# NeuralRevenant/RASSEngine

Measured on NVIDIA B200. Metric: exact top-10 QPS @10M x 1024 (cosine, ids identical to the fp64 CPU oracle), higher is better.
Workload: dtype bf16 scan (fp32 accumulate) + fp64 rerank

## Files before the change

### rassengine_b200/csrc/common.cuh

```cuda
#pragma once
#include <cuda_runtime.h>
#include <cuda_bf16.h>
#include <stdint.h>
#include <stdio.h>
#include <string>
#include <vector>

#include "../../include/rass_b200.h"

#define RASS_WARPS_PER_CTA 8
#define RASS_MAX_K 128
#define RASS_CAND_MAX 2048
#define RASS_GROUP_Q 64
#define RASS_QPAD 256
#define RASS_STREAM_SEG 64
static inline int rass_tc_seg(int k) { return k > 32 ? 512 : 256; }
__host__ __device__ constexpr int rass_tc_keep(int seg) { return seg == 512 ? 128 : seg / 8; }
#define RASS_EXACT_NQ 4
#define RASS_FINISH_THREADS 1024

struct RowMap {
  int64_t base;
  int32_t g, G, blk_log2;
};
// ... 53 lines not shown
  std::vector<int64_t> indptr_host;
  std::vector<float> idf_host;
  std::vector<float> xmin_host, xmax_host;
  bool force_ordered = false;
  bool maxscore = false;
  int* sel_fallback = nullptr;
  std::vector<TextSegment> pending;
  uint32_t* doclen_dev = nullptr;
  uint32_t* gen_dev = nullptr;
  bool has_rewrite = false;
  int doclen_F = 0;
  int64_t doclen_stride = 0;
  std::vector<int64_t> field_vocab;
  std::vector<int64_t> field_last_row;
  bool contiguous_fields = true;
  std::vector<int64_t> field_doc_count, field_sum_ttf;
  std::vector<uint8_t> field_omit_norms;
  int64_t pending_V = 0;
  void* scratch = nullptr;
  size_t scratch_bytes = 0;
};

struct StoreScalars {
  float rho_x;
  float max_xnorm;
  float rho_x8;
};

struct SearchScalars {
  int flagged_n;
  int max_cand;
  int n_certified;
  int finish_done;
  int tile_ctr[2];
};

struct SearchWs {
  SearchScalars* scal = nullptr;
  int q_cap = 0;
  float* q_raw = nullptr;
  float* q_hat = nullptr;
  __nv_bfloat16* q16 = nullptr;
  double* q_norm = nullptr;
  float* q_rho = nullptr;
  int8_t* q8 = nullptr;
  float* q8_scale = nullptr;
  float* q_rho8 = nullptr;
  uint32_t* q_gthr = nullptr;
  size_t pool_entries = 0;
  size_t pool_alloc_entries = 0;
  float* pool_key = nullptr;
  uint32_t* pool_row = nullptr;
  size_t pool_segs = 0;
  size_t pool_alloc_segs = 0;
  float* pool_thr = nullptr;
  int* pool_cnt = nullptr;
  int* flagged = nullptr;
  int* flagged_host = nullptr;
  void* tmap_q = nullptr;
  void* tmap_q2 = nullptr;
  const void* tmap_qbase = nullptr;
  const void* tmap_q2base = nullptr;
  void* tmap_q8 = nullptr;
  const void* tmap_q8base = nullptr;
};

struct VmArray {
  void* base = nullptr;
  size_t reserved = 0, mapped = 0, chunk = 0;
  int device = 0;
  std::vector<unsigned long long> handles;
};
bool vm_available();
bool vm_reserve(VmArray* a, int device, size_t max_bytes, size_t chunk_hint);
int vm_grow(VmArray* a, size_t bytes);
void vm_free(VmArray* a);

struct rass_engine {
  int dim = 0, dim_pad = 0, metric = 0, device = 0;
  uint32_t flags = 0;
  int num_sms = 0;
  int path = RASS_PATH_AUTO;
  int64_t cap = 0, n_rows = 0, n_live = 0;
  RowMap rmap = {0, 0, 1, RASS_SHARD_BLOCK_LOG2};
  struct ShardSet* shards = nullptr;
  float* x32 = nullptr;
  __nv_bfloat16* x16 = nullptr;
  double* norm64 = nullptr;
  float* sa = nullptr;
// ... 201 lines not shown

  __device__ __forceinline__ bool admits_ascending(K k) const { return k > thr_key; }

  __device__ __noinline__ void insert(K k, uint32_t r) {
    if (!entry_better<K>(k, r, thr_key, thr_row)) return;
    const int lane = threadIdx.x & 31;
    int slot = -1;
#pragma unroll
    for (int i = M - 1; i >= 0; --i)
      if (key[i] == thr_key && row[i] == thr_row) slot = i;
    unsigned holders = __ballot_sync(0xffffffffu, slot >= 0);
    int owner = __ffs(holders) - 1;
    if (lane == owner) {
#pragma unroll
      for (int i = 0; i < M; ++i)
        if (i == slot) { key[i] = k; row[i] = r; }
    }
    K wk = key[0];
    uint32_t wr = row[0];
#pragma unroll
    for (int i = 1; i < M; ++i)
      if (entry_better<K>(wk, wr, key[i], row[i])) { wk = key[i]; wr = row[i]; }
#pragma unroll
    for (int m = 16; m >= 1; m >>= 1) {
      K ok = shfl_xor_t(wk, m);
      uint32_t orow = __shfl_xor_sync(0xffffffffu, wr, m);
      if (entry_better<K>(wk, wr, ok, orow)) { wk = ok; wr = orow; }
    }
    thr_key = wk;
    thr_row = wr;
  }
};

template <bool BF16_ROWS>
__device__ __forceinline__ double exact_key_warp(const float* __restrict__ x32, const __nv_bfloat16* __restrict__ x16,
                                                 const double* __restrict__ norm64, uint32_t row, const float* qs,
                                                 double qnorm, int dim_pad, int metric) {
  const int lane = threadIdx.x & 31;
  double acc = 0.0;
  if (BF16_ROWS) {
    const uint4* p = reinterpret_cast<const uint4*>(x16 + (size_t)row * dim_pad);
    for (int j = lane; j < dim_pad / 8; j += 32) {
      uint4 v = __ldg(p + j);
      const uint32_t w[4] = {v.x, v.y, v.z, v.w};
      const float* qq = qs + j * 8;
#pragma unroll
      for (int e = 0; e < 4; ++e) {
        double a = (double)bf16lo(w[e]), b = (double)bf16hi(w[e]);
        double q0 = (double)qq[2 * e], q1 = (double)qq[2 * e + 1];
        if (metric == RASS_METRIC_COSINE) {
          acc = fma(a, q0, acc);
          acc = fma(b, q1, acc);
        } else {
          double d0 = a - q0, d1 = b - q1;
          acc = fma(d0, d0, acc);
          acc = fma(d1, d1, acc);
        }
      }
    }
  } else {
    const float4* p = reinterpret_cast<const float4*>(x32 + (size_t)row * dim_pad);
    for (int j = lane; j < dim_pad / 4; j += 32) {
      float4 v = __ldg(p + j);
      const float4 q = *reinterpret_cast<const float4*>(qs + j * 4);
      if (metric == RASS_METRIC_COSINE) {
        acc = fma((double)v.x, (double)q.x, acc);
        acc = fma((double)v.y, (double)q.y, acc);
        acc = fma((double)v.z, (double)q.z, acc);
        acc = fma((double)v.w, (double)q.w, acc);
      } else {
        double d0 = (double)v.x - (double)q.x, d1 = (double)v.y - (double)q.y;
        double d2 = (double)v.z - (double)q.z, d3 = (double)v.w - (double)q.w;
        acc = fma(d0, d0, acc);
        acc = fma(d1, d1, acc);
        acc = fma(d2, d2, acc);
        acc = fma(d3, d3, acc);
      }
    }
  }
  acc = warp_sum(acc);
  if (metric == RASS_METRIC_COSINE) {
    double den = norm64[row] * qnorm;
    return den > 0.0 ? acc / den : 0.0;
  }
  return -acc;
}

__device__ __forceinline__ float int8_key(int32_t acc1, int32_t acc2, float s1, float s2, float sa8, float sb) {
  return __fmaf_rn(__fmaf_rn(s1, __int2float_rn(acc1), __fmul_rn(s2, __int2float_rn(acc2))), sa8, sb);
}

__device__ __forceinline__ float warp_max_nonneg(float v) {
  return __uint_as_float(__reduce_max_sync(0xffffffffu, __float_as_uint(v)));
}

__device__ __forceinline__ float int8_code(float v, float s) {
  return s > 0.f ? fminf(fmaxf(rintf(__fdiv_rn(v, s)), -127.f), 127.f) : 0.f;
}

__device__ __forceinline__ float score_from_key(double key, int metric) {
  return metric == RASS_METRIC_COSINE ? (float)(1.0 / (2.0 - key)) : (float)(1.0 / (1.0 - key));
}

#endif

int launch_store_convert(rass_engine* h, const float* src_dev, int64_t src_stride, int64_t first_row, int64_t n,
                         cudaStream_t st);
int launch_query_prep(rass_engine* h, const SearchWs& ws, const float* q_dev, int B, cudaStream_t st);
int launch_seed_thresholds(rass_engine* h, const SearchWs& ws, int B, int seg, size_t n_clear, bool* cleared,
// ... 104 lines not shown
```

### rassengine_b200/csrc/engine.cu

```cuda
#include <stdarg.h>
#include <string.h>

#include <algorithm>

#include "common.cuh"

thread_local std::string g_create_error;

int rass_fail(rass_engine* h, int code, const char* fmt, ...) {
  char buf[512];
  va_list ap;
  va_start(ap, fmt);
  vsnprintf(buf, sizeof(buf), fmt, ap);
  va_end(ap);
  if (h) h->err = buf;
  else g_create_error = buf;
  return code;
}

extern "C" const char* rass_version(void) { return "rass-b200 0.1 (abi 1, sm_100a)"; }

extern "C" const char* rass_last_error(const rass_engine* h) { return h ? h->err.c_str() : g_create_error.c_str(); }

#define CHECK_HANDLE(h)                    \
// ... 119 lines not shown
  do {                                                                                              \
    cudaError_t e_ = (call);                                                                        \
    if (e_ != cudaSuccess) {                                                                        \
      h->err = std::string(#call) + " failed: " + cudaGetErrorString(e_);                           \
      return bail(e_ == cudaErrorMemoryAllocation ? RASS_E_OOM : RASS_E_CUDA);                      \
    }                                                                                               \
  } while (0)
  CREATE_TRY(cudaStreamCreateWithFlags(&h->stream, cudaStreamNonBlocking));
  CREATE_TRY(cudaStreamCreateWithFlags(&h->copy_stream, cudaStreamNonBlocking));
  for (int i = 0; i < 4; ++i) CREATE_TRY(cudaEventCreate(&h->ev[i]));
  for (int i = 0; i < 2; ++i) CREATE_TRY(cudaEventCreateWithFlags(&h->stage_ev[i], cudaEventDisableTiming));
  h->stage_bytes = (size_t)32 << 20;
  for (int i = 0; i < 2; ++i) CREATE_TRY(cudaMallocHost(&h->stage[i], h->stage_bytes));
  CREATE_TRY(cudaMalloc(&h->store_scal, sizeof(StoreScalars)));
  CREATE_TRY(cudaMemset(h->store_scal, 0, sizeof(StoreScalars)));
  CREATE_TRY(cudaMalloc(&h->ws[0].scal, sizeof(SearchScalars)));
  CREATE_TRY(cudaMemset(h->ws[0].scal, 0, sizeof(SearchScalars)));
  CREATE_TRY(cudaMallocHost(&h->scal_host, sizeof(SearchScalars)));
  memset(h->scal_host, 0, sizeof(SearchScalars));
#undef CREATE_TRY
  if (capacity_rows > 0) {
    int rc = ensure_capacity(h, capacity_rows);
    if (rc) return bail(rc);
  }
  *out = h;
  return RASS_OK;
}

static void free_search_ws(SearchWs& w) {
  cudaFree(w.scal);
  cudaFree(w.q_raw); cudaFree(w.q_hat); cudaFree(w.q16); cudaFree(w.q_norm); cudaFree(w.q_rho); cudaFree(w.q_gthr);
  cudaFree(w.q8); cudaFree(w.q8_scale); cudaFree(w.q_rho8);
  cudaFree(w.pool_key); cudaFree(w.pool_row); cudaFree(w.pool_thr); cudaFree(w.pool_cnt);
  cudaFree(w.flagged); cudaFreeHost(w.flagged_host);
  free(w.tmap_q); free(w.tmap_q2); free(w.tmap_q8);
}

extern "C" int rass_destroy(rass_engine* h) {
  SHARDED(h, sharded_destroy(h));
  if (!h) return RASS_OK;
  cudaSetDevice(h->device);
  cudaDeviceSynchronize();
  if (h->use_vm) {
    for (int i = 0; i < 7; ++i) vm_free(&h->vm[i]);
  } else {
    cudaFree(h->x32); cudaFree(h->x16); cudaFree(h->norm64); cudaFree(h->sa); cudaFree(h->sb);
    cudaFree(h->x8); cudaFree(h->sa8);
  }
  cudaFree(h->store_scal); cudaFreeHost(h->scal_host);
  for (SearchWs& w : h->ws) free_search_ws(w);
  cudaFree(h->dev_stage);
  cudaFree(h->xlist_key); cudaFree(h->xlist_row);
  cudaFree(h->out_rows); cudaFree(h->out_scores); cudaFree(h->out_keys);
  cudaFreeHost(h->out_rows_host); cudaFreeHost(h->out_scores_host); cudaFreeHost(h->out_keys_host);
  cudaFreeHost(h->q_stage_host);
  cudaFree(h->q_stage_dev);
  cudaFree(h->row_filter);
  cudaFree(h->filter_rows_dev);
  cudaFree(h->flist_dev);
  cudaFree(h->sb_filtered);
  cudaFree(h->retry_ids); cudaFree(h->retry_q); cudaFree(h->retry_rows); cudaFree(h->retry_scores); cudaFree(h->retry_keys);
  for (int i = 0; i < 2; ++i) {
    if (h->slot_stream[i]) cudaStreamDestroy(h->slot_stream[i]);
    if (h->slot_fork[i]) cudaEventDestroy(h->slot_fork[i]);
  }
  for (cudaEvent_t e : h->ev_pool) if (e) cudaEventDestroy(e);
// ... 374 lines not shown
  REALLOC_DEV(h, ws.q_norm, cap);
  REALLOC_DEV(h, ws.q_rho, cap);
  REALLOC_DEV(h, ws.q_gthr, cap);
  if (has_int8_shadow(h->flags)) {
    REALLOC_DEV(h, ws.q8, cap * 2 * d);
    REALLOC_DEV(h, ws.q8_scale, cap * 2);
    REALLOC_DEV(h, ws.q_rho8, cap);
  }
  REALLOC_DEV(h, ws.flagged, cap);
  REALLOC_HOST(h, ws.flagged_host, cap);
  ws.q_cap = (int)cap;
  ws.tmap_qbase = nullptr;
  ws.tmap_q2base = nullptr;
  ws.tmap_q8base = nullptr;
  return RASS_OK;
}

int ensure_pool(rass_engine* h, SearchWs& ws, size_t entries_per_query, size_t segs_per_query, size_t n_queries) {
  const size_t need_e = entries_per_query * n_queries, need_s = segs_per_query * n_queries;
  if (need_e > ws.pool_alloc_entries) {
    { const int rc_ = sync_for_realloc(h); if (rc_) return rc_; }
    ws.pool_alloc_entries = 0;
    REALLOC_DEV(h, ws.pool_key, need_e);
    REALLOC_DEV(h, ws.pool_row, need_e);
    ws.pool_alloc_entries = need_e;
  }
  if (need_s > ws.pool_alloc_segs) {
    { const int rc_ = sync_for_realloc(h); if (rc_) return rc_; }
    ws.pool_alloc_segs = 0;
    REALLOC_DEV(h, ws.pool_thr, need_s);
    REALLOC_DEV(h, ws.pool_cnt, need_s);
    ws.pool_alloc_segs = need_s;
  }
  ws.pool_entries = entries_per_query;
  ws.pool_segs = segs_per_query;
  return RASS_OK;
}

int ensure_xlist_workspace(rass_engine* h, size_t entries) {
  if (entries <= h->xlist_entries) return RASS_OK;
  CUDA_TRY(h, cudaStreamSynchronize(eng_stream(h)));
  REALLOC_DEV(h, h->xlist_key, entries * RASS_EXACT_NQ);
  REALLOC_DEV(h, h->xlist_row, entries * RASS_EXACT_NQ);
  h->xlist_entries = entries;
  return RASS_OK;
}

int ensure_out_workspace(rass_engine* h, size_t n) {
  if (n <= h->out_cap) return RASS_OK;
  CUDA_TRY(h, cudaStreamSynchronize(eng_stream(h)));
  REALLOC_DEV(h, h->out_rows, n);
  REALLOC_DEV(h, h->out_scores, n);
  REALLOC_DEV(h, h->out_keys, n);
  REALLOC_HOST(h, h->out_rows_host, n);
  REALLOC_HOST(h, h->out_scores_host, n);
  REALLOC_HOST(h, h->out_keys_host, n);
  h->out_cap = n;
  return RASS_OK;
}

__global__ void fill_empty_kernel(int64_t* rows, float* scores, double* keys, size_t n) {
  const size_t i = (size_t)blockIdx.x * blockDim.x + threadIdx.x;
  if (i >= n) return;
  rows[i] = -1;
  scores[i] = 0.f;
  if (keys) keys[i] = 0.0;
// ... 126 lines not shown
    s.n_certified = B;
    s.launches = 1;
    if (stats) *stats = s;
    return RASS_OK;
  }
  if ((rc = refresh_store_scalars(h))) return rc;
  int path = resolve_path(h, B, k);
  int64_t* flag_out = as ? async_flag_dev : nullptr;
  if (robust && (path == RASS_PATH_STREAM || path == RASS_PATH_UMMA8)) path = RASS_PATH_UMMA;
  s.path = path;
  if (!(as && h->async_overlap) && (rc = select_scan_offsets(h, st))) return rc;
  if (!as) CUDA_TRY(h, cudaEventRecord(h->ev[0], st));
  if ((rc = launch_query_prep(h, ws, q_dev, B, st))) return rc;
  s.launches = 1;
  size_t n_ev = 0;
  if (path == RASS_PATH_EXACT) {
    for (int i = 0; i < B; ++i) ws.flagged_host[i] = i;
    CUDA_TRY(h, cudaEventRecord(h->ev[1], st));
    if ((rc = launch_exact(h, ws, k, ws.flagged_host, B, out_rows, out_scores, out_keys, st, &s.launches))) return rc;
    s.n_fallback = B;
    s.passes = (B + RASS_EXACT_NQ - 1) / RASS_EXACT_NQ;
    s.bytes_streamed = (int64_t)s.passes * h->n_rows * h->dim_pad * ((h->flags & RASS_BF16_ONLY) ? 2 : 4);
  } else if (path == RASS_PATH_GEMM) {
    const int n_segs = scan_gemm_segs(h, B);
    const int seg = robust ? rass_tc_seg(k) : 256;
    if ((rc = ensure_pool(h, ws, (size_t)n_segs * seg, (size_t)n_segs, (size_t)B))) return rc;
    bool cleared = false;
    if ((rc = launch_seed_thresholds(h, ws, B, seg, (size_t)n_segs * B, &cleared, st))) return rc;
    CUDA_TRY(h, cudaEventRecord(get_event(h, ev_base + n_ev++), st));
    if ((rc = launch_scan_gemm(h, ws, B, seg, st, cleared))) return rc;
    CUDA_TRY(h, cudaEventRecord(get_event(h, ev_base + n_ev++), st));
    if ((rc = launch_finish(h, ws, 0, B, k, n_segs, seg, true, SCAN_BF16, out_rows, out_scores, out_keys, st, flag_out)))
      return rc;
    s.launches += cleared ? 3 : 4;
    s.passes = (B + 255) / 256;
    s.bytes_streamed = (int64_t)s.passes * h->n_rows * h->dim_pad * 2;
  } else {
    const bool int8 = path == RASS_PATH_UMMA8;
    const bool umma = path == RASS_PATH_UMMA || int8;
    const ScanOperands ops = int8 ? SCAN_INT8 : (umma ? SCAN_BF16 : SCAN_FP32_Q);
    const int n_segs = umma ? scan_umma_segs(h) : scan_stream_segs(h);
    const int seg = umma ? (robust ? rass_tc_seg(k) : 256) : RASS_STREAM_SEG;
    if ((rc = ensure_pool(h, ws, (size_t)n_segs * seg, (size_t)n_segs))) return rc;
    bool cleared = false;
    if (umma) {
      if ((rc = launch_seed_thresholds(h, ws, B, seg, (size_t)n_segs * RASS_GROUP_Q, &cleared, st, int8))) return rc;
      s.launches += 1;
    }
    for (int g0 = 0; g0 < B; g0 += RASS_GROUP_Q) {
      const int ng = std::min(RASS_GROUP_Q, B - g0);
      CUDA_TRY(h, cudaEventRecord(get_event(h, ev_base + n_ev++), st));
      if (umma) {
        const bool skip_clear = cleared && g0 == 0;
        if ((rc = launch_scan_umma(h, ws, g0, ng, seg, st, skip_clear, int8))) return rc;
        s.launches += skip_clear ? 1 : 2;
        s.passes += 1;
      } else {
        for (int q0 = g0; q0 < g0 + ng; q0 += 2) {
          if ((rc = launch_scan_stream(h, ws, q0, std::min(2, g0 + ng - q0), g0, st))) return rc;
          s.launches += 1;
          s.passes += 1;
        }
      }
      CUDA_TRY(h, cudaEventRecord(get_event(h, ev_base + n_ev++), st));
      if ((rc = launch_finish(h, ws, g0, ng, k, n_segs, seg, true, ops, out_rows, out_scores, out_keys, st, flag_out)))
        return rc;
      s.launches += 1;
    }
    s.bytes_streamed = (int64_t)s.passes * h->n_rows * h->dim_pad * (int8 ? 1 : 2);
  }
  if (as) {
    if (path == RASS_PATH_EXACT) return rass_fail(h, RASS_E_INVALID, "the fp64 scan has no async form");
    CUDA_TRY(h, cudaMemcpyAsync(as->scal_host, ws.scal, sizeof(SearchScalars), cudaMemcpyDeviceToHost, st));
    CUDA_TRY(h, cudaEventRecord(as->done, st));
    as->stats = s;
    as->k = k;
    as->n_ev = n_ev;
    as->trivial = false;
    as->pending = true;
    return RASS_OK;
  }
  if (path != RASS_PATH_EXACT) {
    CUDA_TRY(h, cudaEventRecord(h->ev[1], st));
    CUDA_TRY(h, cudaMemcpyAsync(h->scal_host, ws.scal, sizeof(SearchScalars), cudaMemcpyDeviceToHost, st));
    CUDA_TRY(h, cudaStreamSynchronize(st));
    const int nf = h->scal_host->flagged_n;
    note_int8_outcome(h, s.path, B, k, nf, robust);
    s.n_certified = h->scal_host->n_certified;
    s.max_candidates = h->scal_host->max_cand;
    if (nf > 0) {
      CUDA_TRY(h, cudaMemcpyAsync(ws.flagged_host, ws.flagged, (size_t)nf * sizeof(int), cudaMemcpyDeviceToHost, st));
      CUDA_TRY(h, cudaStreamSynchronize(st));
      std::sort(ws.flagged_host, ws.flagged_host + nf);
      const bool second_chance = !robust && (path == RASS_PATH_UMMA8 || (k > 32 && rass_tc_seg(k) != 256));
      if (second_chance) {
        float pre = 0.f;
        CUDA_TRY(h, cudaEventElapsedTime(&pre, h->ev[0], h->ev[1]));
        if ((rc = scan_ms_of(h, ev_base, n_ev, &first_scan_ms))) return rc;
        n_ev = 0;
        first_total_ms = pre;
// ... 363 lines not shown
```

### rassengine_b200/csrc/finish.cu

```cuda
#include "common.cuh"

struct FinishArgs {
  const float* pool_key;
  const uint32_t* pool_row;
  const float* pool_thr;
  const int* pool_cnt;
  size_t pool_entries;
  int n_segs, seg_size;
  const float* x32;
  const __nv_bfloat16* x16;
  const double* norm64;
  const float* q_raw;
  const double* q_norm;
  const float* q_rho;
  const StoreScalars* store;
  int int8;
  SearchScalars* scal;
  int* flagged;
  int dim_pad, metric, k, g0;
  float acc_eps;
  RowMap rmap;
  int64_t* out_rows;
  float* out_scores;
  double* out_keys;
  int64_t* flag_out;
};

template <bool BF16_ROWS>
__global__ void __launch_bounds__(RASS_FINISH_THREADS, 1) finish_kernel(FinishArgs a) {
  extern __shared__ __align__(16) unsigned char smem_raw[];
  float* qs = reinterpret_cast<float*>(smem_raw);
  double* ckey = reinterpret_cast<double*>(qs + a.dim_pad);
  uint32_t* crow = reinterpret_cast<uint32_t*>(ckey + RASS_CAND_MAX);
  __shared__ float s_red[32];
  __shared__ int s_redi[32];
  __shared__ float s_t;
  __shared__ int s_valid, s_ncand, s_have;
  __shared__ double s_sk;

  const int tid = threadIdx.x, lane = tid & 31, warp = tid >> 5;
  const int slot = blockIdx.x;
  const int q = a.g0 + slot;
  const float* pk = a.pool_key + (size_t)slot * a.pool_entries;
  const uint32_t* pr = a.pool_row + (size_t)slot * a.pool_entries;

  for (int j = tid; j < a.dim_pad; j += blockDim.x) qs[j] = a.q_raw[(size_t)q * a.dim_pad + j];
  if (tid == 0) { s_ncand = 0; s_have = 0; }

  float mx = neg_inf<float>();
  int nvalid = 0;
  for (int sgm = warp; sgm < a.n_segs; sgm += RASS_FINISH_THREADS / 32) {
    const int cnt = a.pool_cnt ? min(a.pool_cnt[(size_t)slot * a.n_segs + sgm], a.seg_size) : a.seg_size;
    for (int i = lane; i < cnt; i += 32) {
      const size_t o = (size_t)sgm * a.seg_size + i;
      if (a.pool_cnt || pr[o] != 0xffffffffu) {
        ++nvalid;
        mx = fmaxf(mx, pk[o]);
      }
    }
  }
  float t = neg_inf<float>();
  for (int s = tid; s < a.n_segs; s += blockDim.x) t = fmaxf(t, a.pool_thr[(size_t)slot * a.n_segs + s]);
#pragma unroll
  for (int m = 16; m >= 1; m >>= 1) {
    t = fmaxf(t, __shfl_xor_sync(0xffffffffu, t, m));
    nvalid += __shfl_xor_sync(0xffffffffu, nvalid, m);
  }
  if (lane == 0) { s_red[warp] = t; s_redi[warp] = nvalid; }
  __syncthreads();
  if (warp == 0) {
    float tt = s_red[lane];
    int nv = s_redi[lane];
#pragma unroll
    for (int m = 16; m >= 1; m >>= 1) {
      tt = fmaxf(tt, __shfl_xor_sync(0xffffffffu, tt, m));
      nv += __shfl_xor_sync(0xffffffffu, nv, m);
    }
    if (lane == 0) { s_t = tt; s_valid = nv; }
  }

  float bprime;
  {
    const uint32_t mine = mx > neg_inf<float>() ? ord32(mx) : 0u;
    uint32_t prefix = 0;
#pragma unroll 1
    for (int bit = 31; bit >= 0; --bit) {
      const uint32_t cand = prefix | (1u << bit);
      if (__syncthreads_count(mine >= cand) >= a.k) prefix = cand;
    }
    bprime = prefix > 0x007fffffu ? unord32(prefix) : neg_inf<float>();
  }

  float eps;
  {
    const float rho_x = a.int8 ? a.store->rho_x8 : (BF16_ROWS ? 0.f : a.store->rho_x);
    const float rho_q = a.q_rho ? a.q_rho[q] : 0.f;
    float e = rho_x * (1.f + rho_q) + rho_q + a.acc_eps;
    if (a.metric == RASS_METRIC_L2) {
      const float xm = a.store->max_xnorm;
      e = e * xm * (float)a.q_norm[q] * 1.0001f + 6.0e-8f * xm * xm;
    }
    eps = e * 1.0001f;
  }
  const float cutoff = bprime - 2.f * eps;

  for (int sgm = warp; sgm < a.n_segs; sgm += RASS_FINISH_THREADS / 32) {
    const int cnt = a.pool_cnt ? min(a.pool_cnt[(size_t)slot * a.n_segs + sgm], a.seg_size) : a.seg_size;
    for (int i = lane; i < cnt; i += 32) {
      const size_t o = (size_t)sgm * a.seg_size + i;
      if ((a.pool_cnt || pr[o] != 0xffffffffu) && pk[o] >= cutoff) {
        int pos = atomicAdd(&s_ncand, 1);
        if (pos < RASS_CAND_MAX) crow[pos] = pr[o];
      }
    }
  }
  __syncthreads();
  const int ncand_raw = s_ncand;
  const int ncand = min(ncand_raw, RASS_CAND_MAX);

  const double qn = a.q_norm[q];
  for (int c = warp; c < ncand; c += RASS_FINISH_THREADS / 32) {
    double key = exact_key_warp<BF16_ROWS>(a.x32, a.x16, a.norm64, crow[c], qs, qn, a.dim_pad, a.metric);
    if (lane == 0) ckey[c] = key;
  }
  __syncthreads();

  const int kk = a.k;
  for (int c = tid; c < ncand; c += blockDim.x) {
    const double key = ckey[c];
    const uint32_t row = crow[c];
    int rank = 0;
    for (int j = 0; j < ncand; ++j) rank += entry_better<double>(ckey[j], crow[j], key, row);
    if (rank < kk) {
      const size_t o = (size_t)q * kk + rank;
      a.out_rows[o] = row_local_to_global(a.rmap, (int64_t)row);
      a.out_scores[o] = score_from_key(key, a.metric);
      if (a.out_keys) a.out_keys[o] = a.metric == RASS_METRIC_COSINE ? key : -key;
      if (rank == kk - 1) { s_sk = key; s_have = 1; }
    }
  }
  for (int r = ncand + tid; r < kk; r += blockDim.x) {
    const size_t o = (size_t)q * kk + r;
    a.out_rows[o] = -1;
    a.out_scores[o] = 0.f;
    if (a.out_keys) a.out_keys[o] = 0.0;
  }
  __syncthreads();

  if (tid == 0) {
    bool ok;
    const float tt = s_t;
    if (ncand_raw > RASS_CAND_MAX) {
      ok = false;
    } else if (!s_have) {
      ok = (tt == neg_inf<float>()) && ncand == s_valid;
    } else if (tt == neg_inf<float>()) {
      ok = true;
    } else {
      double sk = s_sk;
      if (a.metric == RASS_METRIC_L2) sk = 0.5 * (qn * qn + sk);
      ok = (double)tt + (double)eps < sk;
    }
    if (ok) {
      atomicAdd(&a.scal->n_certified, 1);
    } else {
      int pos = atomicAdd(&a.scal->flagged_n, 1);
      a.flagged[pos] = q;
    }
    atomicMax(&a.scal->max_cand, ncand_raw);
    if (a.flag_out) {
      __threadfence();
      if (atomicAdd(&a.scal->finish_done, 1) == (int)gridDim.x - 1) {
        a.scal->finish_done = 0;
        *a.flag_out = (int64_t)atomicAdd(&a.scal->flagged_n, 0);
      }
    }
  }
}

static size_t finish_smem(int dim_pad) {
  return (size_t)dim_pad * 4 + RASS_CAND_MAX * 12;
}

int launch_finish(rass_engine* h, const SearchWs& ws, int g0, int ng, int k, int n_segs, int seg_size, bool has_cnt,
                  ScanOperands ops, int64_t* out_rows, float* out_scores, double* out_keys, cudaStream_t st,
                  int64_t* flag_out) {
  FinishArgs a;
  a.flag_out = flag_out;
  a.pool_key = ws.pool_key;
  a.pool_row = ws.pool_row;
  a.pool_thr = ws.pool_thr;
  a.pool_cnt = has_cnt ? ws.pool_cnt : nullptr;
  a.pool_entries = ws.pool_entries;
  a.n_segs = n_segs;
  a.seg_size = seg_size;
  a.x32 = h->x32;
  a.x16 = h->x16;
  a.norm64 = h->norm64;
  a.q_raw = ws.q_raw;
  a.q_norm = ws.q_norm;
  a.q_rho = ops == SCAN_INT8 ? ws.q_rho8 : (ops == SCAN_BF16 ? ws.q_rho : nullptr);
  a.int8 = ops == SCAN_INT8;
  a.store = h->store_scal;
  a.scal = ws.scal;
  a.flagged = ws.flagged;
  a.dim_pad = h->dim_pad;
  a.metric = h->metric;
  a.k = k;
  a.g0 = g0;
  a.acc_eps = acc_allowance(h->dim_pad);
  a.rmap = h->rmap;
  a.out_rows = out_rows;
  a.out_scores = out_scores;
  a.out_keys = out_keys;
  const size_t smem = finish_smem(h->dim_pad);
  if (h->flags & RASS_BF16_ONLY) {
    CUDA_TRY(h, cudaFuncSetAttribute(finish_kernel<true>, cudaFuncAttributeMaxDynamicSharedMemorySize, (int)smem));
    finish_kernel<true><<<ng, RASS_FINISH_THREADS, smem, st>>>(a);
  } else {
    CUDA_TRY(h, cudaFuncSetAttribute(finish_kernel<false>, cudaFuncAttributeMaxDynamicSharedMemorySize, (int)smem));
    finish_kernel<false><<<ng, RASS_FINISH_THREADS, smem, st>>>(a);
  }
  CUDA_TRY(h, cudaGetLastError());
  return RASS_OK;
}

template <bool BF16_ROWS, int M>
__global__ void __launch_bounds__(RASS_WARPS_PER_CTA * 32) exact_scan_kernel(
    const float* __restrict__ x32, const __nv_bfloat16* __restrict__ x16, const double* __restrict__ norm64,
    const float* __restrict__ sb, const float* __restrict__ q_raw, const double* __restrict__ q_norm,
    const int* __restrict__ qids, int nq, int64_t n_rows, int dim_pad, int metric, double* __restrict__ xkey,
    uint32_t* __restrict__ xrow, size_t xlist_entries) {
  extern __shared__ __align__(16) unsigned char smem_raw[];
  float* qs = reinterpret_cast<float*>(smem_raw);
  const int lane = threadIdx.x & 31, warp = threadIdx.x >> 5;
  const int gw = blockIdx.x * RASS_WARPS_PER_CTA + warp;
  const int W = gridDim.x * RASS_WARPS_PER_CTA;
  for (int i = threadIdx.x; i < nq * dim_pad; i += blockDim.x)
    qs[i] = q_raw[(size_t)qids[i / dim_pad] * dim_pad + (i % dim_pad)];
  __syncthreads();
  double qn[RASS_EXACT_NQ];
  WarpTop<double, M> top[RASS_EXACT_NQ];
#pragma unroll
  for (int i = 0; i < RASS_EXACT_NQ; ++i) {
    top[i].init();
    qn[i] = i < nq ? q_norm[qids[i]] : 0.0;
  }
  for (int64_t row = gw; row < n_rows; row += W) {
    if (sb[row] == neg_inf<float>()) continue;
#pragma unroll
    for (int i = 0; i < RASS_EXACT_NQ; ++i) {
      if (i < nq) {
        double key = exact_key_warp<BF16_ROWS>(x32, x16, norm64, (uint32_t)row, qs + (size_t)i * dim_pad, qn[i],
                                               dim_pad, metric);
        if (top[i].admits_ascending(key)) top[i].insert(key, (uint32_t)row);
      }
    }
  }
#pragma unroll
  for (int i = 0; i < RASS_EXACT_NQ; ++i) {
    if (i < nq) {
      const size_t base = (size_t)i * xlist_entries + (size_t)gw * (32 * M);
#pragma unroll
      for (int s = 0; s < M; ++s) {
        xkey[base + s * 32 + lane] = top[i].key[s];
        xrow[base + s * 32 + lane] = top[i].row[s];
      }
    }
  }
}

__device__ __forceinline__ uint64_t ord64(double d) {
  if (d == 0.0) d = 0.0;
  uint64_t u = (uint64_t)__double_as_longlong(d);
  return (u >> 63) ? ~u : (u | 0x8000000000000000ULL);
}

__global__ void __launch_bounds__(1024, 1) exact_select_kernel(const double* __restrict__ xkey,
                                                               const uint32_t* __restrict__ xrow, size_t xlist_entries,
                                                               int n, int k, const int* __restrict__ qids, int q_fixed,
                                                               int raw_score, int metric,
                                                               RowMap rmap, int64_t* __restrict__ out_rows,
                                                               float* __restrict__ out_scores,
                                                               double* __restrict__ out_keys,
                                                               const int* __restrict__ only_if) {
  if (only_if && !only_if[blockIdx.x]) return;
  __shared__ int hist[256];
  __shared__ int s_bucket, s_remaining, s_nsel, s_nvalid;
  __shared__ double selk[RASS_MAX_K];
  __shared__ uint32_t selr[RASS_MAX_K];
  const int tid = threadIdx.x;
  const int q = qids ? qids[blockIdx.x] : q_fixed + (int)blockIdx.x;
  const double* key = xkey + (size_t)blockIdx.x * xlist_entries;
  const uint32_t* row = xrow + (size_t)blockIdx.x * xlist_entries;

  if (tid == 0) { s_nvalid = 0; s_nsel = 0; }
  __syncthreads();
  int nv = 0;
  for (int i = tid; i < n; i += blockDim.x) nv += row[i] != 0xffffffffu;
  if (nv) atomicAdd(&s_nvalid, nv);
  __syncthreads();
  const int kk = min(k, s_nvalid);

  uint64_t pre_hi = 0, mask_hi = 0;
  uint32_t pre_lo = 0, mask_lo = 0;
  if (kk > 0) {
    if (tid == 0) s_remaining = kk;
    for (int byte = 11; byte >= 0; --byte) {
// ... 178 lines not shown
```

### rassengine_b200/csrc/store.cu

```cuda
#include <cooperative_groups.h>

#include "common.cuh"

__global__ void __launch_bounds__(256) store_convert_kernel(const float* __restrict__ src, int64_t src_stride, int dim,
                                                            int dim_pad, int metric, int bf16_only, int write32,
                                                            float* __restrict__ x32, __nv_bfloat16* __restrict__ x16,
                                                            double* __restrict__ norm64, float* __restrict__ sa,
                                                            float* __restrict__ sb, int8_t* __restrict__ x8,
                                                            float* __restrict__ sa8, StoreScalars* scal,
                                                            int64_t first_row, int64_t n) {
  const int lane = threadIdx.x & 31;
  const int64_t r = (int64_t)blockIdx.x * (blockDim.x >> 5) + (threadIdx.x >> 5);
  if (r >= n) return;
  const int64_t row = first_row + r;
  const float* s = src + r * src_stride;
  double n2 = 0.0, e2 = 0.0;
  float amax = 0.f;
  for (int j = lane * 4; j < dim_pad; j += 128) {
    float v[4];
#pragma unroll
    for (int e = 0; e < 4; ++e) {
      v[e] = (j + e < dim) ? s[j + e] : 0.f;
      amax = fmaxf(amax, fabsf(v[e]));
    }
// ... 55 lines not shown
    atomicMax(reinterpret_cast<int*>(&scal->rho_x8), __float_as_int(rho));
  }
}

int launch_store_convert(rass_engine* h, const float* src_dev, int64_t src_stride, int64_t first_row, int64_t n,
                         cudaStream_t st) {
  if (n <= 0) return RASS_OK;
  h->sb_filtered_dirty = true;
  h->store_scal_stale = true;
  const bool bf16_only = (h->flags & RASS_BF16_ONLY) != 0;
  const bool in_place = !bf16_only && src_dev == h->x32 + (size_t)first_row * h->dim_pad;
  const int warps = 8;
  int64_t blocks = (n + warps - 1) / warps;
  store_convert_kernel<<<(unsigned)blocks, warps * 32, 0, st>>>(src_dev, src_stride, h->dim, h->dim_pad, h->metric,
                                                                bf16_only ? 1 : 0, (!bf16_only && !in_place) ? 1 : 0,
                                                                h->x32, h->x16, h->norm64, h->sa, h->sb, h->x8, h->sa8,
                                                                h->store_scal, first_row, n);
  CUDA_TRY(h, cudaGetLastError());
  return RASS_OK;
}

__global__ void __launch_bounds__(128) query_prep_kernel(const float* __restrict__ q, int dim, int dim_pad, int metric,
                                                         int B, int B_pad, float* __restrict__ q_raw,
                                                         float* __restrict__ q_hat, __nv_bfloat16* __restrict__ q16,
                                                         double* __restrict__ q_norm, float* __restrict__ q_rho,
                                                         int8_t* __restrict__ q8, float* __restrict__ q8_scale,
                                                         float* __restrict__ q_rho8, SearchScalars* __restrict__ scal) {
  const int lane = threadIdx.x & 31;
  const int b = blockIdx.x * (blockDim.x >> 5) + (threadIdx.x >> 5);
  if (blockIdx.x == 0 && threadIdx.x == 0) {
    scal->flagged_n = 0;
    scal->max_cand = 0;
    scal->n_certified = 0;
    scal->tile_ctr[0] = 0;
    scal->tile_ctr[1] = 0;
  }
  if (b >= B_pad) return;
  const size_t r1 = (size_t)(b / RASS_GROUP_Q) * (2 * RASS_GROUP_Q) + (b % RASS_GROUP_Q), r2 = r1 + RASS_GROUP_Q;
  if (b >= B) {
    for (int j = lane; j < dim_pad; j += 32) q16[(size_t)b * dim_pad + j] = __float2bfloat16_rn(0.f);
    if (q8) {
      for (int j = lane; j < dim_pad; j += 32) { q8[r1 * dim_pad + j] = 0; q8[r2 * dim_pad + j] = 0; }
      if (lane < 2) q8_scale[2 * b + lane] = 0.f;
    }
    return;
  }
  const float* s = q + (size_t)b * dim;
  double n2 = 0.0;
  for (int j = lane; j < dim; j += 32) n2 = fma((double)s[j], (double)s[j], n2);
  n2 = warp_sum(n2);
  const double nrm = sqrt(n2);
  const double inv = (metric == RASS_METRIC_COSINE) ? (nrm > 0.0 ? 1.0 / nrm : 0.0) : 1.0;
  double h2 = 0.0, e2 = 0.0;
  float amax = 0.f;
  for (int j = lane; j < dim_pad; j += 32) {
    float v = j < dim ? s[j] : 0.f;
    float hat = (float)((double)v * inv);
    amax = fmaxf(amax, fabsf(hat));
    __nv_bfloat16 hb = __float2bfloat16_rn(hat);
    double d = (double)hat - (double)__bfloat162float(hb);
    h2 = fma((double)hat, (double)hat, h2);
    e2 = fma(d, d, e2);
    q_raw[(size_t)b * dim_pad + j] = v;
    q_hat[(size_t)b * dim_pad + j] = hat;
    q16[(size_t)b * dim_pad + j] = hb;
  }
// ... 245 lines not shown
```

Measured before the change: 35270.

## Split finish into collect, grid-wide rerank, and radix select kernels

The single per-query finish kernel becomes three kernels. The first collects candidate rows per query into a global list. The second spreads the fp64 exact-key rerank of all candidates across every SM, instead of tying it to one 1024-thread CTA per query. The third does a radix threshold select followed by ranking only the survivors, replacing an O(ncand^2) rank. The exact-key loop also batches 8 loads per lane and the exact scan gets a min-blocks launch bound, at the cost of two extra launches and global candidate buffers.

Measured after the change: 35530, median of 6. Within noise of the previous version (+0.7%).

```diff
diff --git a/rassengine_b200/csrc/common.cuh b/rassengine_b200/csrc/common.cuh
--- a/rassengine_b200/csrc/common.cuh
+++ b/rassengine_b200/csrc/common.cuh
@@ -109,7 +109,16 @@
   int max_cand;
   int n_certified;
   int finish_done;
+  int cand_total;
   int tile_ctr[2];
+};
+
+struct FinishQuery {
+  float t;
+  float eps;
+  int valid;
+  int ncand;
+  int base;
 };
 
 struct SearchWs {
@@ -132,6 +141,10 @@
   size_t pool_alloc_segs = 0;
   float* pool_thr = nullptr;
   int* pool_cnt = nullptr;
+  size_t cand_slots = 0;
+  uint2* cand_list = nullptr;
+  double* cand_key = nullptr;
+  FinishQuery* cand_q = nullptr;
   int* flagged = nullptr;
   int* flagged_host = nullptr;
   void* tmap_q = nullptr;
@@ -399,6 +412,7 @@
   }
 };
 
+#define EXACT_KEY_LOADS 8
 template <bool BF16_ROWS>
 __device__ __forceinline__ double exact_key_warp(const float* __restrict__ x32, const __nv_bfloat16* __restrict__ x16,
                                                  const double* __restrict__ norm64, uint32_t row, const float* qs,
@@ -407,41 +421,59 @@
   double acc = 0.0;
   if (BF16_ROWS) {
     const uint4* p = reinterpret_cast<const uint4*>(x16 + (size_t)row * dim_pad);
-    for (int j = lane; j < dim_pad / 8; j += 32) {
-      uint4 v = __ldg(p + j);
-      const uint32_t w[4] = {v.x, v.y, v.z, v.w};
-      const float* qq = qs + j * 8;
-#pragma unroll
-      for (int e = 0; e < 4; ++e) {
-        double a = (double)bf16lo(w[e]), b = (double)bf16hi(w[e]);
-        double q0 = (double)qq[2 * e], q1 = (double)qq[2 * e + 1];
-        if (metric == RASS_METRIC_COSINE) {
-          acc = fma(a, q0, acc);
-          acc = fma(b, q1, acc);
-        } else {
-          double d0 = a - q0, d1 = b - q1;
-          acc = fma(d0, d0, acc);
-          acc = fma(d1, d1, acc);
+    const int n = dim_pad / 8;
+    for (int j0 = lane; j0 < n; j0 += 32 * EXACT_KEY_LOADS) {
+      uint4 v[EXACT_KEY_LOADS];
+#pragma unroll
+      for (int u = 0; u < EXACT_KEY_LOADS; ++u)
+        if (j0 + 32 * u < n) v[u] = __ldg(p + j0 + 32 * u);
+#pragma unroll
+      for (int u = 0; u < EXACT_KEY_LOADS; ++u) {
+        const int j = j0 + 32 * u;
+        if (j >= n) break;
+        const uint32_t w[4] = {v[u].x, v[u].y, v[u].z, v[u].w};
+        const float* qq = qs + j * 8;
+#pragma unroll
+        for (int e = 0; e < 4; ++e) {
+          double a = (double)bf16lo(w[e]), b = (double)bf16hi(w[e]);
+          double q0 = (double)qq[2 * e], q1 = (double)qq[2 * e + 1];
+          if (metric == RASS_METRIC_COSINE) {
+            acc = fma(a, q0, acc);
+            acc = fma(b, q1, acc);
+          } else {
+            double d0 = a - q0, d1 = b - q1;
+            acc = fma(d0, d0, acc);
+            acc = fma(d1, d1, acc);
+          }
         }
       }
     }
   } else {
     const float4* p = reinterpret_cast<const float4*>(x32 + (size_t)row * dim_pad);
-    for (int j = lane; j < dim_pad / 4; j += 32) {
-      float4 v = __ldg(p + j);
-      const float4 q = *reinterpret_cast<const float4*>(qs + j * 4);
-      if (metric == RASS_METRIC_COSINE) {
-        acc = fma((double)v.x, (double)q.x, acc);
-        acc = fma((double)v.y, (double)q.y, acc);
-        acc = fma((double)v.z, (double)q.z, acc);
-        acc = fma((double)v.w, (double)q.w, acc);
-      } else {
-        double d0 = (double)v.x - (double)q.x, d1 = (double)v.y - (double)q.y;
-        double d2 = (double)v.z - (double)q.z, d3 = (double)v.w - (double)q.w;
-        acc = fma(d0, d0, acc);
-        acc = fma(d1, d1, acc);
-        acc = fma(d2, d2, acc);
-        acc = fma(d3, d3, acc);
+    const int n = dim_pad / 4;
+    for (int j0 = lane; j0 < n; j0 += 32 * EXACT_KEY_LOADS) {
+      float4 v[EXACT_KEY_LOADS];
+#pragma unroll
+      for (int u = 0; u < EXACT_KEY_LOADS; ++u)
+        if (j0 + 32 * u < n) v[u] = __ldg(p + j0 + 32 * u);
+#pragma unroll
+      for (int u = 0; u < EXACT_KEY_LOADS; ++u) {
+        const int j = j0 + 32 * u;
+        if (j >= n) break;
+        const float4 q = *reinterpret_cast<const float4*>(qs + j * 4);
+        if (metric == RASS_METRIC_COSINE) {
+          acc = fma((double)v[u].x, (double)q.x, acc);
+          acc = fma((double)v[u].y, (double)q.y, acc);
+          acc = fma((double)v[u].z, (double)q.z, acc);
+          acc = fma((double)v[u].w, (double)q.w, acc);
+        } else {
+          double d0 = (double)v[u].x - (double)q.x, d1 = (double)v[u].y - (double)q.y;
+          double d2 = (double)v[u].z - (double)q.z, d3 = (double)v[u].w - (double)q.w;
+          acc = fma(d0, d0, acc);
+          acc = fma(d1, d1, acc);
+          acc = fma(d2, d2, acc);
+          acc = fma(d3, d3, acc);
+        }
       }
     }
   }
diff --git a/rassengine_b200/csrc/engine.cu b/rassengine_b200/csrc/engine.cu
--- a/rassengine_b200/csrc/engine.cu
+++ b/rassengine_b200/csrc/engine.cu
@@ -175,6 +175,7 @@
   cudaFree(w.q_raw); cudaFree(w.q_hat); cudaFree(w.q16); cudaFree(w.q_norm); cudaFree(w.q_rho); cudaFree(w.q_gthr);
   cudaFree(w.q8); cudaFree(w.q8_scale); cudaFree(w.q_rho8);
   cudaFree(w.pool_key); cudaFree(w.pool_row); cudaFree(w.pool_thr); cudaFree(w.pool_cnt);
+  cudaFree(w.cand_list); cudaFree(w.cand_key); cudaFree(w.cand_q);
   cudaFree(w.flagged); cudaFreeHost(w.flagged_host);
   free(w.tmap_q); free(w.tmap_q2); free(w.tmap_q8);
 }
@@ -615,6 +616,14 @@
     REALLOC_DEV(h, ws.pool_cnt, need_s);
     ws.pool_alloc_segs = need_s;
   }
+  if (n_queries > ws.cand_slots) {
+    { const int rc_ = sync_for_realloc(h); if (rc_) return rc_; }
+    ws.cand_slots = 0;
+    REALLOC_DEV(h, ws.cand_list, n_queries * RASS_CAND_MAX);
+    REALLOC_DEV(h, ws.cand_key, n_queries * RASS_CAND_MAX);
+    REALLOC_DEV(h, ws.cand_q, n_queries);
+    ws.cand_slots = n_queries;
+  }
   ws.pool_entries = entries_per_query;
   ws.pool_segs = segs_per_query;
   return RASS_OK;
@@ -807,7 +816,7 @@
     CUDA_TRY(h, cudaEventRecord(get_event(h, ev_base + n_ev++), st));
     if ((rc = launch_finish(h, ws, 0, B, k, n_segs, seg, true, SCAN_BF16, out_rows, out_scores, out_keys, st, flag_out)))
       return rc;
-    s.launches += cleared ? 3 : 4;
+    s.launches += cleared ? 5 : 6;
     s.passes = (B + 255) / 256;
     s.bytes_streamed = (int64_t)s.passes * h->n_rows * h->dim_pad * 2;
   } else {
@@ -840,7 +849,7 @@
       CUDA_TRY(h, cudaEventRecord(get_event(h, ev_base + n_ev++), st));
       if ((rc = launch_finish(h, ws, g0, ng, k, n_segs, seg, true, ops, out_rows, out_scores, out_keys, st, flag_out)))
         return rc;
-      s.launches += 1;
+      s.launches += 3;
     }
     s.bytes_streamed = (int64_t)s.passes * h->n_rows * h->dim_pad * (int8 ? 1 : 2);
   }
diff --git a/rassengine_b200/csrc/finish.cu b/rassengine_b200/csrc/finish.cu
--- a/rassengine_b200/csrc/finish.cu
+++ b/rassengine_b200/csrc/finish.cu
@@ -15,42 +15,50 @@
   const float* q_rho;
   const StoreScalars* store;
   int int8;
+  int bf16_rows;
   SearchScalars* scal;
   int* flagged;
   int dim_pad, metric, k, g0;
   float acc_eps;
   RowMap rmap;
+  uint2* cand_list;
+  double* cand_key;
+  FinishQuery* cand_q;
   int64_t* out_rows;
   float* out_scores;
   double* out_keys;
   int64_t* flag_out;
 };
 
-template <bool BF16_ROWS>
-__global__ void __launch_bounds__(RASS_FINISH_THREADS, 1) finish_kernel(FinishArgs a) {
-  extern __shared__ __align__(16) unsigned char smem_raw[];
-  float* qs = reinterpret_cast<float*>(smem_raw);
-  double* ckey = reinterpret_cast<double*>(qs + a.dim_pad);
-  uint32_t* crow = reinterpret_cast<uint32_t*>(ckey + RASS_CAND_MAX);
+__device__ __forceinline__ uint64_t ord64(double d) {
+  if (d == 0.0) d = 0.0;
+  uint64_t u = (uint64_t)__double_as_longlong(d);
+  return (u >> 63) ? ~u : (u | 0x8000000000000000ULL);
+}
+
+__global__ void __launch_bounds__(RASS_FINISH_THREADS, 1) finish_collect_kernel(FinishArgs a) {
+  __shared__ uint32_t crow[RASS_CAND_MAX];
   __shared__ float s_red[32];
   __shared__ int s_redi[32];
   __shared__ float s_t;
-  __shared__ int s_valid, s_ncand, s_have;
-  __shared__ double s_sk;
+  __shared__ int s_valid, s_ncand, s_base;
 
   const int tid = threadIdx.x, lane = tid & 31, warp = tid >> 5;
   const int slot = blockIdx.x;
   const int q = a.g0 + slot;
   const float* pk = a.pool_key + (size_t)slot * a.pool_entries;
   const uint32_t* pr = a.pool_row + (size_t)slot * a.pool_entries;
-
-  for (int j = tid; j < a.dim_pad; j += blockDim.x) qs[j] = a.q_raw[(size_t)q * a.dim_pad + j];
-  if (tid == 0) { s_ncand = 0; s_have = 0; }
+  auto seg_count = [&](int sgm) {
+    return sgm >= a.n_segs ? 0 : (a.pool_cnt ? min(a.pool_cnt[(size_t)slot * a.n_segs + sgm], a.seg_size) : a.seg_size);
+  };
+
+  if (tid == 0) s_ncand = 0;
 
   float mx = neg_inf<float>();
   int nvalid = 0;
+  int cnt = seg_count(warp);
   for (int sgm = warp; sgm < a.n_segs; sgm += RASS_FINISH_THREADS / 32) {
-    const int cnt = a.pool_cnt ? min(a.pool_cnt[(size_t)slot * a.n_segs + sgm], a.seg_size) : a.seg_size;
+    const int cnt_next = seg_count(sgm + RASS_FINISH_THREADS / 32);
     for (int i = lane; i < cnt; i += 32) {
       const size_t o = (size_t)sgm * a.seg_size + i;
       if (a.pool_cnt || pr[o] != 0xffffffffu) {
@@ -58,6 +66,7 @@
         mx = fmaxf(mx, pk[o]);
       }
     }
+    cnt = cnt_next;
   }
   float t = neg_inf<float>();
   for (int s = tid; s < a.n_segs; s += blockDim.x) t = fmaxf(t, a.pool_thr[(size_t)slot * a.n_segs + s]);
@@ -93,7 +102,7 @@
 
   float eps;
   {
-    const float rho_x = a.int8 ? a.store->rho_x8 : (BF16_ROWS ? 0.f : a.store->rho_x);
+    const float rho_x = a.int8 ? a.store->rho_x8 : (a.bf16_rows ? 0.f : a.store->rho_x);
     const float rho_q = a.q_rho ? a.q_rho[q] : 0.f;
     float e = rho_x * (1.f + rho_q) + rho_q + a.acc_eps;
     if (a.metric == RASS_METRIC_L2) {
@@ -104,8 +113,9 @@
   }
   const float cutoff = bprime - 2.f * eps;
 
+  cnt = seg_count(warp);
   for (int sgm = warp; sgm < a.n_segs; sgm += RASS_FINISH_THREADS / 32) {
-    const int cnt = a.pool_cnt ? min(a.pool_cnt[(size_t)slot * a.n_segs + sgm], a.seg_size) : a.seg_size;
+    const int cnt_next = seg_count(sgm + RASS_FINISH_THREADS / 32);
     for (int i = lane; i < cnt; i += 32) {
       const size_t o = (size_t)sgm * a.seg_size + i;
       if ((a.pool_cnt || pr[o] != 0xffffffffu) && pk[o] >= cutoff) {
@@ -113,30 +123,114 @@
         if (pos < RASS_CAND_MAX) crow[pos] = pr[o];
       }
     }
-  }
-  __syncthreads();
-  const int ncand_raw = s_ncand;
+    cnt = cnt_next;
+  }
+  __syncthreads();
+  const int ncand = min(s_ncand, RASS_CAND_MAX);
+  if (tid == 0) {
+    s_base = atomicAdd(&a.scal->cand_total, ncand);
+    a.cand_q[slot] = FinishQuery{s_t, eps, s_valid, s_ncand, s_base};
+    atomicMax(&a.scal->max_cand, s_ncand);
+  }
+  __syncthreads();
+  for (int i = tid; i < ncand; i += blockDim.x) a.cand_list[s_base + i] = make_uint2(crow[i], (uint32_t)slot);
+}
+
+#define RASS_RERANK_THREADS 256
+#define RASS_RERANK_CTAS_PER_SM 4
+template <bool BF16_ROWS>
+__global__ void __launch_bounds__(RASS_RERANK_THREADS, RASS_RERANK_CTAS_PER_SM) finish_rerank_kernel(FinishArgs a) {
+  constexpr int WARPS = RASS_RERANK_THREADS / 32;
+  const int lane = threadIdx.x & 31;
+  const int n = a.scal->cand_total;
+  const int per_cta = (n + (int)gridDim.x - 1) / (int)gridDim.x;
+  const int end = min(n, ((int)blockIdx.x + 1) * per_cta);
+  int i = (int)blockIdx.x * per_cta + (threadIdx.x >> 5);
+  uint2 next = i < end ? a.cand_list[i] : make_uint2(0, 0);
+  for (; i < end; i += WARPS) {
+    const uint2 cur = next;
+    if (i + WARPS < end) next = a.cand_list[i + WARPS];
+    const int q = a.g0 + (int)cur.y;
+    const double key = exact_key_warp<BF16_ROWS>(a.x32, a.x16, a.norm64, cur.x, a.q_raw + (size_t)q * a.dim_pad,
+                                                 a.q_norm[q], a.dim_pad, a.metric);
+    if (lane == 0) a.cand_key[i] = key;
+  }
+}
+
+#define RASS_SELECT_THREADS 256
+__global__ void __launch_bounds__(RASS_SELECT_THREADS) finish_select_kernel(FinishArgs a) {
+  constexpr int E = RASS_CAND_MAX / RASS_SELECT_THREADS;
+  constexpr int WARPS = RASS_SELECT_THREADS / 32;
+  static_assert(E * RASS_SELECT_THREADS == RASS_CAND_MAX, "every candidate has one thread");
+  __shared__ double skey[RASS_CAND_MAX];
+  __shared__ uint32_t srow[RASS_CAND_MAX];
+  __shared__ int s_cnt[2][WARPS];
+  __shared__ int s_nsel, s_have;
+  __shared__ double s_sk;
+
+  const int tid = threadIdx.x, lane = tid & 31, warp = tid >> 5;
+  const int slot = blockIdx.x, q = a.g0 + slot;
+  const FinishQuery fq = a.cand_q[slot];
+  const int ncand_raw = fq.ncand;
   const int ncand = min(ncand_raw, RASS_CAND_MAX);
-
-  const double qn = a.q_norm[q];
-  for (int c = warp; c < ncand; c += RASS_FINISH_THREADS / 32) {
-    double key = exact_key_warp<BF16_ROWS>(a.x32, a.x16, a.norm64, crow[c], qs, qn, a.dim_pad, a.metric);
-    if (lane == 0) ckey[c] = key;
-  }
-  __syncthreads();
-
   const int kk = a.k;
-  for (int c = tid; c < ncand; c += blockDim.x) {
-    const double key = ckey[c];
-    const uint32_t row = crow[c];
+
+  double key[E];
+  uint32_t row[E];
+  uint64_t ok[E];
+#pragma unroll
+  for (int e = 0; e < E; ++e) {
+    const int i = tid + e * RASS_SELECT_THREADS;
+    key[e] = 0.0;
+    row[e] = 0;
+    ok[e] = 0;
+    if (i < ncand) {
+      key[e] = a.cand_key[fq.base + i];
+      row[e] = a.cand_list[fq.base + i].x;
+      ok[e] = ord64(key[e]);
+    }
+  }
+  if (tid == 0) { s_nsel = 0; s_have = 0; }
+  __syncthreads();
+
+  uint64_t T = 0;
+  int have = ncand;
+#pragma unroll 1
+  for (int bit = 63; bit >= 0 && have > kk; --bit) {
+    const uint64_t c = T | (1ull << bit);
+    int m = 0;
+#pragma unroll
+    for (int e = 0; e < E; ++e) m += ok[e] >= c;
+    m = __reduce_add_sync(0xffffffffu, m);
+    if (lane == 0) s_cnt[bit & 1][warp] = m;
+    __syncthreads();
+    int cnt = 0;
+#pragma unroll
+    for (int w = 0; w < WARPS; ++w) cnt += s_cnt[bit & 1][w];
+    if (cnt >= kk) { T = c; have = cnt; }
+  }
+#pragma unroll
+  for (int e = 0; e < E; ++e) {
+    if (ok[e] != 0 && ok[e] >= T) {
+      const int pos = atomicAdd(&s_nsel, 1);
+      skey[pos] = key[e];
+      srow[pos] = row[e];
+    }
+  }
+  __syncthreads();
+
+  const int nsel = s_nsel;
+  for (int c = tid; c < nsel; c += blockDim.x) {
+    const double kc = skey[c];
+    const uint32_t rc = srow[c];
     int rank = 0;
-    for (int j = 0; j < ncand; ++j) rank += entry_better<double>(ckey[j], crow[j], key, row);
+    for (int j = 0; j < nsel; ++j) rank += entry_better<double>(skey[j], srow[j], kc, rc);
     if (rank < kk) {
       const size_t o = (size_t)q * kk + rank;
-      a.out_rows[o] = row_local_to_global(a.rmap, (int64_t)row);
-      a.out_scores[o] = score_from_key(key, a.metric);
-      if (a.out_keys) a.out_keys[o] = a.metric == RASS_METRIC_COSINE ? key : -key;
-      if (rank == kk - 1) { s_sk = key; s_have = 1; }
+      a.out_rows[o] = row_local_to_global(a.rmap, (int64_t)rc);
+      a.out_scores[o] = score_from_key(kc, a.metric);
+      if (a.out_keys) a.out_keys[o] = a.metric == RASS_METRIC_COSINE ? kc : -kc;
+      if (rank == kk - 1) { s_sk = kc; s_have = 1; }
     }
   }
   for (int r = ncand + tid; r < kk; r += blockDim.x) {
@@ -149,17 +243,20 @@
 
   if (tid == 0) {
     bool ok;
-    const float tt = s_t;
+    const float tt = fq.t;
     if (ncand_raw > RASS_CAND_MAX) {
       ok = false;
     } else if (!s_have) {
-      ok = (tt == neg_inf<float>()) && ncand == s_valid;
+      ok = (tt == neg_inf<float>()) && ncand == fq.valid;
     } else if (tt == neg_inf<float>()) {
       ok = true;
     } else {
       double sk = s_sk;
-      if (a.metric == RASS_METRIC_L2) sk = 0.5 * (qn * qn + sk);
-      ok = (double)tt + (double)eps < sk;
+      if (a.metric == RASS_METRIC_L2) {
+        const double qn = a.q_norm[q];
+        sk = 0.5 * (qn * qn + sk);
+      }
+      ok = (double)tt + (double)fq.eps < sk;
     }
     if (ok) {
       atomicAdd(&a.scal->n_certified, 1);
@@ -167,24 +264,20 @@
       int pos = atomicAdd(&a.scal->flagged_n, 1);
       a.flagged[pos] = q;
     }
-    atomicMax(&a.scal->max_cand, ncand_raw);
-    if (a.flag_out) {
-      __threadfence();
-      if (atomicAdd(&a.scal->finish_done, 1) == (int)gridDim.x - 1) {
-        a.scal->finish_done = 0;
-        *a.flag_out = (int64_t)atomicAdd(&a.scal->flagged_n, 0);
-      }
-    }
-  }
-}
-
-static size_t finish_smem(int dim_pad) {
-  return (size_t)dim_pad * 4 + RASS_CAND_MAX * 12;
+    __threadfence();
+    if (atomicAdd(&a.scal->finish_done, 1) == (int)gridDim.x - 1) {
+      a.scal->finish_done = 0;
+      a.scal->cand_total = 0;
+      if (a.flag_out) *a.flag_out = (int64_t)atomicAdd(&a.scal->flagged_n, 0);
+    }
+  }
 }
 
 int launch_finish(rass_engine* h, const SearchWs& ws, int g0, int ng, int k, int n_segs, int seg_size, bool has_cnt,
                   ScanOperands ops, int64_t* out_rows, float* out_scores, double* out_keys, cudaStream_t st,
                   int64_t* flag_out) {
+  if ((size_t)ng > ws.cand_slots)
+    return rass_fail(h, RASS_E_INVALID, "finish of %d queries: the rerank workspace holds %zu", ng, ws.cand_slots);
   FinishArgs a;
   a.flag_out = flag_out;
   a.pool_key = ws.pool_key;
@@ -201,6 +294,8 @@
   a.q_norm = ws.q_norm;
   a.q_rho = ops == SCAN_INT8 ? ws.q_rho8 : (ops == SCAN_BF16 ? ws.q_rho : nullptr);
   a.int8 = ops == SCAN_INT8;
+  const bool bf16_rows = (h->flags & RASS_BF16_ONLY) != 0;
+  a.bf16_rows = bf16_rows;
   a.store = h->store_scal;
   a.scal = ws.scal;
   a.flagged = ws.flagged;
@@ -210,23 +305,25 @@
   a.g0 = g0;
   a.acc_eps = acc_allowance(h->dim_pad);
   a.rmap = h->rmap;
+  a.cand_list = ws.cand_list;
+  a.cand_key = ws.cand_key;
+  a.cand_q = ws.cand_q;
   a.out_rows = out_rows;
   a.out_scores = out_scores;
   a.out_keys = out_keys;
-  const size_t smem = finish_smem(h->dim_pad);
-  if (h->flags & RASS_BF16_ONLY) {
-    CUDA_TRY(h, cudaFuncSetAttribute(finish_kernel<true>, cudaFuncAttributeMaxDynamicSharedMemorySize, (int)smem));
-    finish_kernel<true><<<ng, RASS_FINISH_THREADS, smem, st>>>(a);
-  } else {
-    CUDA_TRY(h, cudaFuncSetAttribute(finish_kernel<false>, cudaFuncAttributeMaxDynamicSharedMemorySize, (int)smem));
-    finish_kernel<false><<<ng, RASS_FINISH_THREADS, smem, st>>>(a);
-  }
+  finish_collect_kernel<<<ng, RASS_FINISH_THREADS, 0, st>>>(a);
+  CUDA_TRY(h, cudaGetLastError());
+  const int grid = h->num_sms * RASS_RERANK_CTAS_PER_SM;
+  if (bf16_rows) finish_rerank_kernel<true><<<grid, RASS_RERANK_THREADS, 0, st>>>(a);
+  else finish_rerank_kernel<false><<<grid, RASS_RERANK_THREADS, 0, st>>>(a);
+  CUDA_TRY(h, cudaGetLastError());
+  finish_select_kernel<<<ng, RASS_SELECT_THREADS, 0, st>>>(a);
   CUDA_TRY(h, cudaGetLastError());
   return RASS_OK;
 }
 
 template <bool BF16_ROWS, int M>
-__global__ void __launch_bounds__(RASS_WARPS_PER_CTA * 32) exact_scan_kernel(
+__global__ void __launch_bounds__(RASS_WARPS_PER_CTA * 32, 2) exact_scan_kernel(
     const float* __restrict__ x32, const __nv_bfloat16* __restrict__ x16, const double* __restrict__ norm64,
     const float* __restrict__ sb, const float* __restrict__ q_raw, const double* __restrict__ q_norm,
     const int* __restrict__ qids, int nq, int64_t n_rows, int dim_pad, int metric, double* __restrict__ xkey,
@@ -268,12 +365,6 @@
       }
     }
   }
-}
-
-__device__ __forceinline__ uint64_t ord64(double d) {
-  if (d == 0.0) d = 0.0;
-  uint64_t u = (uint64_t)__double_as_longlong(d);
-  return (u >> 63) ? ~u : (u | 0x8000000000000000ULL);
 }
 
 __global__ void __launch_bounds__(1024, 1) exact_select_kernel(const double* __restrict__ xkey,
diff --git a/rassengine_b200/csrc/store.cu b/rassengine_b200/csrc/store.cu
--- a/rassengine_b200/csrc/store.cu
+++ b/rassengine_b200/csrc/store.cu
@@ -111,6 +111,7 @@
     scal->flagged_n = 0;
     scal->max_cand = 0;
     scal->n_certified = 0;
+    scal->cand_total = 0;
     scal->tile_ctr[0] = 0;
     scal->tile_ctr[1] = 0;
   }
```
